# mit-acl/mppi_numba

Measured on AMD Instinct MI355X. Metric: rollouts/sec (MPPI iteration = noise + rollout + update), higher is better.
Workload: dtype f64 intermediates / f32 state (the reference CPU path's roundings)

## Files before the change

### include/mppi_hip.h

```cpp
#ifndef MPPI_HIP_H
#define MPPI_HIP_H

#include <stdint.h>

#ifdef __cplusplus
extern "C" {
#endif

#define MPPI_HIP_ABI_VERSION 1

typedef enum mppi_status {
  MPPI_OK = 0,
  MPPI_ERR_INVALID = -1,
  MPPI_ERR_HIP = -2,
  MPPI_ERR_STATE = -3,
  MPPI_ERR_NO_DEVICE = -4,
  MPPI_ERR_COMM = -5,
  MPPI_ERR_BUSY = -6
} mppi_status;

typedef enum mppi_mode {
  MPPI_MODE_DET = 0,
  MPPI_MODE_SPEED_MAP = 1,
  MPPI_MODE_TDM = 2,
// ... 166 lines not shown
int mppi_planner_time_kernels(mppi_planner* p, mppi_tdm* lin, mppi_tdm* ang, int reps, float* us_rollout,
                              float* us_update);
int mppi_planner_last_elapsed_ms(mppi_planner* p, float* ms);

int mppi_trace_ranges_enabled(void);

int mppi_planner_describe_last_rollout(mppi_planner* p, char* buf, int capacity);

#define MPPI_DEBUG_NO_SPEC_KERNEL 1
#define MPPI_DEBUG_NO_SPECULATION 2
#define MPPI_DEBUG_NO_DEEP_KERNEL 4
#define MPPI_DEBUG_CC_GLOBAL 8
#define MPPI_DEBUG_KEEP_SPECULATING 16
#define MPPI_DEBUG_NO_SCAN_KERNEL 32
#define MPPI_DEBUG_SCAN_READ_NOISE 64
#define MPPI_DEBUG_SCAN_FULL_TILES 128
#define MPPI_DEBUG_NO_FOLDED_APPLY 256
#define MPPI_DEBUG_NO_REDUCE_FOLD 512
#define MPPI_DEBUG_NO_SCAN_DIRECT 1024
#define MPPI_DEBUG_DROP_NOISE_FLAG 2048
int mppi_planner_set_debug_flags(mppi_planner* p, int flags);
int mppi_planner_set_fold_poll_limit(mppi_planner* p, int polls);
int mppi_planner_fold_state(mppi_planner* p, int* folding, long* faults);
int mppi_debug_occupy_cus(int device, int workgroups, int milliseconds);
int mppi_selftest_philox(int device, int* mismatches);
int mppi_debug_read_stamps(unsigned long long* out, int count, int clear);
int mppi_planner_set_graph_replay(mppi_planner* p, int iterations_per_graph);
int mppi_planner_graph_stats(mppi_planner* p, long* captures, long* replays);
int mppi_planner_graph_probe(mppi_planner* p, mppi_tdm* lin, mppi_tdm* ang, int iterations, int replays,
                             float* us_direct, float* us_graph);

typedef struct mppi_world mppi_world;
int mppi_world_create(int device, int rows, int cols, double res, double xlo, double ylo, const double* lin,
                      const double* ang, mppi_world** out);
int mppi_world_destroy(mppi_world* w);
int mppi_world_get(mppi_world* w, const double* xy, int count, double* lin_out, double* ang_out);
int mppi_world_get_grids(mppi_world* w, double* lin, double* ang);
int mppi_world_sample_true_dist(mppi_world* w, const int32_t* terrain_of_cell, int n_terrains, const double* lin_pool,
                                const double* ang_pool, int pool_len, uint64_t seed);
int mppi_planner_closed_loop(mppi_planner* p, mppi_tdm* lin, mppi_tdm* ang, mppi_world* w, int max_steps,
                             double dt, double goal_tolerance, const double* x_init, double* xhist, float* uhist,
                             int* steps_taken);

#define MPPI_COMM_ID_BYTES 128
int mppi_comm_unique_id(char id[MPPI_COMM_ID_BYTES]);
int mppi_planner_comm_init(mppi_planner* p, const char id[MPPI_COMM_ID_BYTES]);
// ... 25 lines not shown
```

### mppi_numba_amd/_lib.py

```python
import ctypes as C
import os

_HERE = os.path.dirname(os.path.abspath(__file__))
LIB_PATH = os.environ.get("MPPI_HIP_LIB") or os.path.join(_HERE, "libmppi_hip.so")

MPPI_OK = 0
MODE_DET, MODE_SPEED_MAP, MODE_TDM, MODE_BAREBONE = 0, 1, 2, 3
RNG_PHILOX, RNG_XOROSHIRO = 0, 1
MATH_EXACT, MATH_FAST = 0, 1
COMM_ID_BYTES = 128
PREP_TDM, PREP_DET, PREP_SPEED = 0, 1, 2
DEBUG_NO_SPEC_KERNEL, DEBUG_NO_SPECULATION, DEBUG_NO_DEEP_KERNEL, DEBUG_CC_GLOBAL = 1, 2, 4, 8
DEBUG_KEEP_SPECULATING = 16
DEBUG_NO_SCAN_KERNEL, DEBUG_SCAN_READ_NOISE, DEBUG_SCAN_FULL_TILES = 32, 64, 128
DEBUG_NO_FOLDED_APPLY = 256
DEBUG_NO_REDUCE_FOLD = 512
DEBUG_NO_SCAN_DIRECT = 1024
DEBUG_DROP_NOISE_FLAG = 2048
ABI_VERSION = 1
P2P_HANDLE_BYTES = 64


class MppiError(RuntimeError):
    def __init__(self, code, message):
# ... 88 lines not shown
    "mppi_planner_iterate_async": [_vp, _vp, _vp, C.c_int],
    "mppi_planner_synchronize": [_vp],
    "mppi_planner_sample_noise": [_vp],
    "mppi_planner_set_noise": [_vp, _f32p],
    "mppi_planner_get_noise": [_vp, _f32p],
    "mppi_planner_rollout": [_vp, _vp, _vp],
    "mppi_planner_set_costs": [_vp, _f32p],
    "mppi_planner_get_costs": [_vp, _f32p],
    "mppi_planner_get_sample_costs": [_vp, _f32p],
    "mppi_planner_update": [_vp],
    "mppi_planner_get_weights": [_vp, _f32p],
    "mppi_planner_get_state_rollout": [_vp, _vp, _vp, _f32p],
    "mppi_planner_get_instance_state_rollout": [_vp, _vp, _vp, C.c_int, _f32p],
    "mppi_planner_set_instances": [_vp, C.c_int, _f32p, _f32p],
    "mppi_planner_rng_states": [_vp, _u64p, C.c_long, C.POINTER(C.c_long)],
    "mppi_planner_set_profiling": [_vp, C.c_int],
    "mppi_planner_stage_times": [_vp, _f32p],
    "mppi_planner_last_elapsed_ms": [_vp, _f32p],
    "mppi_planner_time_kernels": [_vp, _vp, _vp, C.c_int, _f32p, _f32p],
    "mppi_planner_describe_last_rollout": [_vp, C.c_char_p, C.c_int],
    "mppi_planner_set_debug_flags": [_vp, C.c_int],
    "mppi_planner_set_fold_poll_limit": [_vp, C.c_int],
    "mppi_planner_fold_state": [_vp, C.POINTER(C.c_int), C.POINTER(C.c_long)],
    "mppi_debug_occupy_cus": [C.c_int, C.c_int, C.c_int],
    "mppi_selftest_philox": [C.c_int, C.POINTER(C.c_int)],
    "mppi_debug_read_stamps": [C.POINTER(C.c_ulonglong), C.c_int, C.c_int],
    "mppi_planner_graph_probe": [_vp, _vp, _vp, C.c_int, C.c_int, _f32p, _f32p],
    "mppi_planner_set_graph_replay": [_vp, C.c_int],
    "mppi_planner_graph_stats": [_vp, C.POINTER(C.c_long), C.POINTER(C.c_long)],
    "mppi_planner_p2p_export": [_vp, C.c_char_p],
    "mppi_planner_p2p_connect": [_vp, C.c_char_p, C.c_int],
    "mppi_group_p2p_connect": [C.POINTER(_vp), C.c_int],
    "mppi_planner_p2p_stats": [_vp, C.POINTER(C.c_int), C.POINTER(C.c_long), C.c_char_p, C.c_int],
    "mppi_planner_p2p_set_enabled": [_vp, C.c_int],
    "mppi_planner_p2p_ping": [_vp, C.c_ulonglong, C.c_int, C.POINTER(C.c_int)],
    "mppi_world_create": [C.c_int, C.c_int, C.c_int, C.c_double, C.c_double, C.c_double, _f64p, _f64p, C.POINTER(_vp)],
    "mppi_world_destroy": [_vp],
    "mppi_world_get": [_vp, _f64p, C.c_int, _f64p, _f64p],
    "mppi_world_get_grids": [_vp, _f64p, _f64p],
    "mppi_world_sample_true_dist": [_vp, C.POINTER(C.c_int32), C.c_int, _f64p, _f64p, C.c_int, C.c_uint64],
    "mppi_planner_closed_loop": [_vp, _vp, _vp, _vp, C.c_int, C.c_double, C.c_double, _f64p, _f64p, _f32p, C.POINTER(C.c_int)],
    "mppi_tdm_set_sample_shard": [_vp, C.c_int],
    "mppi_planner_set_sample_sharding": [_vp, C.c_int, C.c_int],
    "mppi_planner_sample_costs_local": [_vp, _f32p],
    "mppi_planner_sample_costs_apply": [_vp, _f32p, C.c_int],
    "mppi_comm_unique_id": [C.c_char_p],
# ... 60 lines not shown
```

### mppi_numba_amd/csrc/handles.h

```cpp
#pragma once
#include "host_common.h"
#include "map_plan.h"

struct mppi_tdm {
  mppi_tdm_cfg cfg;
  hipStream_t stream = nullptr;
  int8_t* grid = nullptr;
  int8_t* pmf = nullptr;
  size_t pmf_capacity = 0;
  int8_t* table = nullptr;
  int table_capacity = 0;
  int8_t* obs = nullptr;
  int8_t* unk = nullptr;
  int8_t* risk = nullptr;
  size_t map_capacity = 0;
  int8_t* raw = nullptr;
  size_t raw_capacity = 0;
  float* bin_values = nullptr;
  int bin_values_capacity = 0;
  int* prep_flags = nullptr;
  uint64_t* states = nullptr;
  long n_states = 0;
  int bins = 0, rows = 0, cols = 0;
  bool has_risk = false, maps_set = false, one_hot = false;
// ... 85 lines not shown
  float2* u = nullptr;
  float2* u_prev = nullptr;
  float2* u_alt = nullptr;
  bool apply_pending = false;
  uint64_t folded_applies = 0;
  float* costs = nullptr;
  float* weights_out = nullptr;
  float* w_rel = nullptr;
  float* tile_beta = nullptr;
  int n_tiles = 0;
  bool tile_packets_fresh = false;
  bool theta_bounded = false;
  float* tile_packets[2] = {nullptr, nullptr};
  int tpk_cur = 0;
  int scan_tile = 32;
  bool scan_packets_fresh = false;
  unsigned long long* published = nullptr;
  unsigned int* fold_fault_host = nullptr;
  unsigned int* fold_fault_dev = nullptr;
  int fold_max_polls = 1 << 20;
  long iterations_since_wait = 0;
  bool fold_off = false;
  uint64_t fold_faults = 0;
  bool reduce_pending = false;
  int reduce_index = 0;
  uint64_t reduced_applies = 0;
  uint64_t bumps_owed = 0;
  bool scan_gen_now = false;
  bool noise_virtual = false;
  int noise_virtual_back = 1;
  double* packets = nullptr;
  double* stats = nullptr;
  uint32_t* cells = nullptr;
  size_t cells_capacity = 0;
  double* cc_scratch = nullptr;
  uint16_t* cells16 = nullptr;
  size_t cells16_capacity = 0;
  int pitch16 = 0;
  bool cells16_valid = false;
  bool cells16_with_risk = false;
  int num_cus = 256;
  int lds_per_cu = 160 * 1024;
  float* sample_costs = nullptr;
  bool want_sample_costs = false;
  uint64_t* states = nullptr;
  long n_states = 0;
// ... 123 lines not shown
```

### mppi_numba_amd/csrc/launch_plan.h

```cpp
#pragma once
#include "handles.h"

static int tdm_max_byte(const mppi_tdm* t) { return t->injected ? (int)t->injected_max : t->table_max; }

static int check_tdms(const mppi_planner* p, const mppi_tdm* lin, const mppi_tdm* ang) {
  if (p->cfg.mode == MPPI_MODE_BAREBONE) return MPPI_OK;
  REQUIRE(lin && ang, MPPI_ERR_INVALID, "lin/ang TDM required in this mode");
  REQUIRE(lin->maps_set && ang->maps_set, MPPI_ERR_STATE, "TDM maps not set");
  REQUIRE(lin->cfg.device == p->cfg.device && ang->cfg.device == p->cfg.device, MPPI_ERR_INVALID,
          "planner and TDMs live on different devices");
  REQUIRE(lin->rows == ang->rows && lin->cols == ang->cols, MPPI_ERR_INVALID,
          "lin and ang TDMs differ in padded size (%dx%d vs %dx%d)", lin->rows, lin->cols, ang->rows,
          ang->cols);
  REQUIRE(lin->cfg.num_grids == p->cfg.num_grid_samples && ang->cfg.num_grids == p->cfg.num_grid_samples,
          MPPI_ERR_INVALID, "TDM num_grids (%d, %d) != planner num_grid_samples (%d)", lin->cfg.num_grids,
          ang->cfg.num_grids, p->cfg.num_grid_samples);
  REQUIRE(lin->cfg.max_rows == ang->cfg.max_rows && lin->cfg.max_cols == ang->cfg.max_cols, MPPI_ERR_INVALID,
          "lin and ang TDMs differ in max_map_dim");
  REQUIRE(p->cfg.mode != MPPI_MODE_SPEED_MAP || lin->has_risk, MPPI_ERR_STATE,
          "speed-map mode needs lin TDM's risk traction map");
  return MPPI_OK;
}

static DevParams make_dev_params(const mppi_planner* p) {
// ... 362 lines not shown
  if (p->apply_pending || p->reduce_pending) {
    const mppi_params& a = p->params;
    pend.packets = p->packets;
    pend.u_out = p->u_alt;
    pend.u_prev = p->u_prev;
    pend.stats = p->stats;
    pend.world = p->cfg.world_size;
    pend.stride = p->B * packet_len(T);
    pend.lambda = a.lambda_weight;
    pend.v_lo = a.vrange[0]; pend.v_hi = a.vrange[1];
    pend.w_lo = a.wrange[0]; pend.w_hi = a.wrange[1];
  }
  if (p->reduce_pending) {
    REQUIRE(!p->apply_pending, MPPI_ERR_STATE, "internal: tile packets left to a launch that cannot reduce them");
    REQUIRE(tiles_can_reduce(tiles, T) && plan.tile == p->scan_tile, MPPI_ERR_STATE, "internal: %d workgroups cannot combine the tile packets of %d steps", tiles, T);
    pend.packets = p->packets;
    pend.world = 1;
    pend.reduce_tiles = p->tile_packets[p->tpk_cur];
    pend.reduce_n_tiles = ceil_div(N, p->scan_tile);
    pend.published = p->published;
    pend.flag_set = p->reduce_index & 1;
    pend.fault = p->fold_fault_dev;
    pend.max_polls = p->fold_max_polls;
    if (p->p2p_on) pend.peers = make_peer_exchange(p);
  }
  if (!plan.direct) p->spec_launches += 1;
  REQUIRE(!plan.direct || plan.fallback_offset >= 0, MPPI_ERR_STATE, "internal: direct exact schedule without its map window");
  const ScanFallback fallback = {plan.fallback_offset, plan.fallback_map_bytes, plan.direct ? 1 : 0, plan.rot_ok ? 1 : 0, plan.small_offset};
#define MPPI_LAUNCH_SCAN_EXACT(P2, GEN)                                                                    \
  do {                                                                                                    \
    auto kern = speed ? k_rollout_scan_exact<P2, GEN, false, true>                                        \
                      : (plan.direct ? k_rollout_scan_exact<P2, GEN, true> : k_rollout_scan_exact<P2, GEN, false>); \
    if (plan.lds > 64 * 1024)                                                                             \
      HIP_TRY(hipFuncSetAttribute(reinterpret_cast<const void*>(kern),                                    \
                                  hipFuncAttributeMaxDynamicSharedMemorySize, (int)plan.lds));            \
    MPPI_KLAUNCH(kern, dim3(tiles), dim3(64 * plan.waves), plan.lds, p->stream, d, p->cells16, p->cells,   \
                 p->noise, gen_job, p->u, p->costs, p->w_rel, pk, pend, fallback,                          \
                 (const int8_t*)(speed ? p->packed.risk : nullptr));                                       \
  } while (0)
#define MPPI_LAUNCH_SCAN(RR, P2, GEN)                                                                      \
  do {                                                                                                    \
    auto kern = k_rollout_scan<RR, P2, GEN>;                                                              \
    if (plan.lds > 64 * 1024)                                                                             \
      HIP_TRY(hipFuncSetAttribute(reinterpret_cast<const void*>(kern),                                    \
                                  hipFuncAttributeMaxDynamicSharedMemorySize, (int)plan.lds));            \
    MPPI_KLAUNCH(kern, dim3(tiles + extra), dim3(64 * plan.waves), plan.lds, p->stream, d, p->cells16,    \
// ... 697 lines not shown
```

### mppi_numba_amd/csrc/mppi_api.hip

```cpp
#include "../../include/mppi_hip.h"

#include <dlfcn.h>
#include <hip/hip_runtime.h>
#include <hip/hip_ext.h>
#include <rccl/rccl.h>

#include <algorithm>
#include <atomic>
#include <cmath>
#include <cstdarg>
#include <cstdio>
#include <cstdlib>
#include <cstring>
#include <ctime>
#include <string>
#include <vector>

#include "rng_kernels.h"
#include "rollout_kernels.h"
#include "rollout_crowd_kernel.h"
#include "fleet_kernels.h"
#include "rollout_scan_kernel.h"
#include "rollout_scan_exact_kernel.h"
#include "map_kernels.h"
// ... 437 lines not shown
  if (p->comm && g_rccl.CommDestroy) (void)g_rccl.CommDestroy(p->comm);
  for (int g = 0; g < kMaxFoldedRanks; ++g)
    if (p->peer_mapped[g] && p->peer_inbox[g]) (void)hipIpcCloseMemHandle(p->peer_inbox[g]);
  if (p->inbox) (void)hipFree(p->inbox);
  if (p->p2p_fault_host) (void)hipHostFree(p->p2p_fault_host);
  if (p->fold_fault_host) (void)hipHostFree(p->fold_fault_host);
  dev_free(p->inst_dev);
  if (p->u_host) (void)hipHostFree(p->u_host);
  if (p->u_stage) (void)hipHostFree(p->u_stage);
  if (p->ev_u_staged) (void)hipEventDestroy(p->ev_u_staged);
  dev_free(p->noise_buf[0]);
  dev_free(p->noise_buf[1]);
  dev_free(p->staging);
  dev_free(p->u);
  dev_free(p->u_prev);
  dev_free(p->u_alt);
  dev_free(p->costs);
  dev_free(p->weights_out);
  dev_free(p->w_rel);
  dev_free(p->tile_beta);
  dev_free(p->tile_packets[0]);
  dev_free(p->tile_packets[1]);
  dev_free(p->published);
  dev_free(p->packets);
  dev_free(p->stats);
  dev_free(p->cells);
  dev_free(p->cells16);
  dev_free(p->cc_scratch);
  dev_free(p->sample_costs);
  dev_free(p->states);
  dev_free(p->obs_pos);
  dev_free(p->obs_r);
  dev_free(p->inst_obs_pos);
  dev_free(p->inst_obs_r);
  dev_free(p->trk_pos);
  dev_free(p->trk_pos_rows);
  dev_free(p->trk_r);
  dev_free(p->wall_seg);
  dev_free(p->wall_hw);
  dev_free(p->wtrk_seg_rows);
  dev_free(p->wtrk_hw);
  dev_free(p->wtrk_range);
  dev_free(p->fleet_seg_rows);
  dev_free(p->fleet_hw);
  dev_free(p->fleet_range);
  dev_free(p->fleet_plan);
// ... 68 lines not shown
  HIP_TRY(hipHostMalloc(reinterpret_cast<void**>(&p->u_host), B * T * sizeof(float2), hipHostMallocMapped));
  HIP_TRY(hipHostGetDevicePointer(reinterpret_cast<void**>(&p->u_host_dev), p->u_host, 0));
  memset(p->u_host, 0, B * T * sizeof(float2));
  HIP_TRY(hipHostMalloc(reinterpret_cast<void**>(&p->u_stage), B * T * sizeof(float2), hipHostMallocDefault));
  HIP_TRY(hipEventCreateWithFlags(&p->ev_u_staged, hipEventDisableTiming));
  p->inst_host.assign(B, BatchInst{});
  TRY(dev_alloc(&p->costs, N));
  TRY(dev_alloc(&p->weights_out, N));
  p->n_tiles = ceil_div((long)N, 64);
  TRY(dev_alloc(&p->w_rel, N));
  TRY(dev_alloc(&p->tile_beta, (size_t)p->n_tiles));
  TRY(dev_alloc(&p->packets, (size_t)c.world_size * B * packet_len((int)T)));
  if (c.mode == MPPI_MODE_DET || c.mode == MPPI_MODE_SPEED_MAP) {
    const size_t tiles = (size_t)ceil_div((long)N, 32);
    for (int b = 0; b < 2; ++b) {
      TRY(dev_alloc(&p->tile_packets[b], tiles * (size_t)tile_packet_floats((int)T)));
      HIP_TRY(hipMemsetAsync(p->tile_packets[b], 0, tiles * (size_t)tile_packet_floats((int)T) * sizeof(float), p->stream));
    }
    TRY(dev_alloc(&p->published, published_words((int)T)));
    HIP_TRY(hipMemsetAsync(p->published, 0xff, sizeof(unsigned long long) * published_words((int)T), p->stream));
    HIP_TRY(hipHostMalloc((void**)&p->fold_fault_host, sizeof(unsigned int), hipHostMallocMapped));
    HIP_TRY(hipHostGetDevicePointer((void**)&p->fold_fault_dev, p->fold_fault_host, 0));
    *p->fold_fault_host = 0u;
  }
  TRY(dev_alloc(&p->stats, 2 * B));
  TRY(dev_alloc(&p->state_rollout, (size_t)c.num_vis_state_rollouts * (T + 1) * 3));
  HIP_TRY(hipMemsetAsync(p->u, 0, B * T * sizeof(float2), p->stream));
  HIP_TRY(hipMemsetAsync(p->u_prev, 0, B * T * sizeof(float2), p->stream));
  HIP_TRY(hipMemsetAsync(p->u_alt, 0, B * T * sizeof(float2), p->stream));
  HIP_TRY(hipMemsetAsync(p->costs, 0, N * sizeof(float), p->stream));
  {
    std::vector<double> initial_stats(2 * B);
    for (size_t b = 0; b < B; ++b) { initial_stats[2 * b] = 0.0; initial_stats[2 * b + 1] = 1.0; }
    HIP_TRY(hipMemcpy(p->stats, initial_stats.data(), sizeof(double) * 2 * B, hipMemcpyHostToDevice));
  }
  if (c.rng == MPPI_RNG_XOROSHIRO) {
    long total = (long)c.num_control_rollouts * (long)B * c.num_steps;
    std::vector<uint64_t> host(2 * (size_t)total);
    xoroshiro_init_host(host.data(), total, c.seed);
    p->n_states = (long)N * (long)T;
    TRY(dev_alloc(&p->states, 2 * (size_t)p->n_states));
    HIP_TRY(hipMemcpy(p->states, host.data() + 2 * (size_t)p->n_offset * T,
                      2 * sizeof(uint64_t) * (size_t)p->n_states, hipMemcpyHostToDevice));
  }
  HIP_TRY(hipStreamSynchronize(p->stream));
  return MPPI_OK;
// ... 242 lines not shown
extern "C" int mppi_planner_synchronize(mppi_planner* p) {
  REQUIRE(p, MPPI_ERR_INVALID, "NULL planner");
  HIP_TRY(hipSetDevice(p->cfg.device));
  TRY(wait_for_stream(p));
  TRY(after_drain(p));
  return finish_timing(p);
}

extern "C" int mppi_planner_set_fold_poll_limit(mppi_planner* p, int polls) {
  REQUIRE(p && polls >= 1, MPPI_ERR_INVALID, "bad argument");
  p->fold_max_polls = polls;
  drop_graphs(p);
  p->fold_off = false;
  return MPPI_OK;
}

extern "C" int mppi_planner_fold_state(mppi_planner* p, int* folding, long* faults) {
  REQUIRE(p && folding && faults, MPPI_ERR_INVALID, "NULL argument");
  *folding = p->fold_off ? 0 : 1;
  *faults = (long)p->fold_faults;
  return MPPI_OK;
}

__global__ __launch_bounds__(64) void k_debug_occupy(unsigned long long ticks, int* sink) {
  extern __shared__ int occupy_lds[];
  occupy_lds[threadIdx.x] = (int)threadIdx.x;
  const unsigned long long t0 = wall_clock64();
  while (wall_clock64() - t0 < ticks) __builtin_amdgcn_s_sleep(32);
  if (sink && occupy_lds[threadIdx.x ^ 1] == -1) *sink = 1;
}

extern "C" int mppi_debug_occupy_cus(int device, int workgroups, int milliseconds) {
  REQUIRE(workgroups >= 1 && workgroups <= 4096 && milliseconds >= 1 && milliseconds <= 2000, MPPI_ERR_INVALID, "bad argument");
  HIP_TRY(hipSetDevice(device));
  static hipStream_t sides[64] = {};
  REQUIRE(device >= 0 && device < 64, MPPI_ERR_INVALID, "device %d", device);
  hipStream_t& side = sides[device];
  if (!side) {
    int least = 0, greatest = 0;
    HIP_TRY(hipDeviceGetStreamPriorityRange(&least, &greatest));
    HIP_TRY(hipStreamCreateWithPriority(&side, hipStreamNonBlocking, greatest));
  }
  int rate_khz = 0;
  HIP_TRY(hipDeviceGetAttribute(&rate_khz, hipDeviceAttributeWallClockRate, device));
  if (rate_khz <= 0) rate_khz = 100000;
  const size_t lds = 100 * 1024;
// ... 1107 lines not shown
```

### mppi_numba_amd/csrc/rollout_scan_exact_kernel.h

```cpp
#pragma once
#include "rollout_scan_kernel.h"

namespace mppi {

#ifndef MPPI_SCAN_POLL_SLEEP
#define MPPI_SCAN_POLL_SLEEP 2
#endif

struct ScanFallback {
  int offset;
  int map_bytes;
  int direct;
  int rot_ok;
  int small_offset;
};
static_assert(ScanFallbackLds::kRingBytes == PipeRing<8>::kBytesPerPair, "the region holds one chunk ring of 8 steps");

template <bool POW2RES, typename Background>
__device__ __forceinline__ float scan_exact_reexecute(const DevParams& P, const uint16_t* __restrict__ cells16, char* fb,
                                                      int map_bytes, const float2* e2, const float2* u_src, int T,
                                                      int c, int lane, const float2* us_ready, bool rot_ok,
                                                      Background&& background, bool leave_when_idle = false) {
  constexpr int C = 8, R = ScanExactLds::R;
  using Ring = PipeRing<C>;
// ... 140 lines not shown
#pragma unroll
  for (int i = 0; i < 16; ++i) {
    g = c == i ? kGroupOfWave[i] : g;
    prio = c == i ? kPrioOfWave[i] : prio;
  }
  g = g < W ? g : -1;
  const int k = 2 * g + h;
  [[maybe_unused]] const bool stamp_wg = blockIdx.x == 5 || blockIdx.x == 200;
  [[maybe_unused]] const int stamp_base = (blockIdx.x == 200 ? 1024 : 64) + 16 * c;
  MPPI_STAMP(stamp_wg && c < 16, stamp_base + 0);
  DevParams Q = P;
  const int tile = blockIdx.x;
  const float2* uq = select_instance(Q, u, Q.inst ? (tile * R) / Q.n_inst : 0);
  const int T = Q.n_steps, N = Q.n_local;
  const int Tp = 8 * W;
  const int n = tile * R + r;
  const bool live = n < N;
  const int t0 = k * CHL;
  const int nvalid = min(max(T - t0, 0), CHL);
  const bool folded = pend.packets != nullptr;
  const bool reducing = folded && pend.reduce_tiles != nullptr;
  const int red_t = tile + max(walker, 0) * (int)gridDim.x;
  const bool reduce_here = reducing && (walker == 0 || walker == 1) && red_t < T;
  StepLoads red_loads;
  float2 red_u = make_float2(0.0f, 0.0f);
  if (reduce_here) {
    red_loads = combine_step_issue(pend.reduce_tiles, pend.reduce_n_tiles, tile_packet_floats(T), red_t, lane);
    red_u = uq[red_t];
  }

  const uint32_t ref = scan_lookup<POW2RES, SPEED>(Q, cells16, Q.x0, Q.y0) & 0x3fffu;

  char* base = reinterpret_cast<char*>(scan_lds);
  constexpr bool direct = DIRECT;
  if (direct && c >= 5)
    copy_window_to_lds_direct(Q, cells16, reinterpret_cast<uint16_t*>(base + fallback.offset + (size_t)Tp * 8), 320, (int)blockDim.x - 320);
  float2* e2 = reinterpret_cast<float2*>(base);
  double* ccr = reinterpret_cast<double*>(base + L::e2(W));
  char* grp = base + L::e2(W) + L::ccr(W);
  float2* pos = reinterpret_cast<float2*>(grp + L::grp(W));
  float* th_sh = reinterpret_cast<float*>(pos) + (size_t)Tp * R;
  char* small = DIRECT ? base + fallback.small_offset : reinterpret_cast<char*>(pos) + L::p2(W);
  double2* uos = reinterpret_cast<double2*>(small);
  double* term_sh = reinterpret_cast<double*>(uos + Tp);
  uint32_t* evw = reinterpret_cast<uint32_t*>(term_sh + R);
  float* wsh = reinterpret_cast<float*>(evw + 2 * R);
  uint32_t* flags = reinterpret_cast<uint32_t*>(wsh + R);
  double* scale_sh = reinterpret_cast<double*>(small + (size_t)Tp * 16 + R * 64 + 64);
  float2* u_sh = reinterpret_cast<float2*>(scale_sh + kMaxFoldedRanks + 2);
  int* a_done = reinterpret_cast<int*>(u_sh + Tp);
  int* th_done = a_done + 16;
  int* b_done = th_done + 16;
  int* xy_done = b_done + 16;
  int* ev_done = xy_done + 16;
  int* c_done = ev_done + 16;
  int* cc_done = c_done + 16;
  int* u_ready = cc_done + 16;
  double2* stop_sh = reinterpret_cast<double2*>(u_ready + 16);
  if (c == 4) {
    if (lane < R) {
      evw[2 * lane] = 0u;
      evw[2 * lane + 1] = 0u;
      if (lane == 0) flags[0] = 0u;
    }
    for (int i = lane; i < 8 * 16; i += 64) a_done[i] = 0;
  }
  if (!reducing || c == 1 || (walker < 0 && g < 0)) {
    if (direct && reducing && c >= 5) asm volatile("s_waitcnt vmcnt(0)" ::: "memory");
    lds_barrier();
  }
  MPPI_STAMP(stamp_wg && c < 16, stamp_base + 9);
  auto raise = [&](int* flag, int value) {
    pin_memory_order();
    if (lane == 0) __hip_atomic_store(flag, value, __ATOMIC_RELAXED, __HIP_MEMORY_SCOPE_WORKGROUP);
    pin_memory_order();
  };
  auto peek = [&](const int* flag) {
    return __builtin_amdgcn_readfirstlane(__hip_atomic_load(flag, __ATOMIC_ACQUIRE, __HIP_MEMORY_SCOPE_WORKGROUP));
  };
#ifdef MPPI_POLL_BOUND
  constexpr int kMaxPolls = 1 << 19;
#endif
  auto wait_for = [&](const int* flag) {
    int v;
    [[maybe_unused]] int polls = 0;
    while ((v = peek(flag)) == 0) {
      __builtin_amdgcn_s_sleep(MPPI_SCAN_POLL_SLEEP);
#ifdef MPPI_POLL_BOUND
      if (++polls > kMaxPolls) __builtin_trap();
#endif
    }
    return v;
  };
  const double dt64 = (double)Q.dt;

  if (folded && (walker == 0 || walker == 1)) {
    __builtin_amdgcn_s_setprio(3);
    if (reducing) {
      MPPI_STAMP(stamp_wg, stamp_base + 5);
      if (reduce_here) {
        const int stride = tile_packet_floats(T);
        publish_step(pend, combine_step_finish(red_loads, pend.reduce_tiles, pend.reduce_n_tiles, stride, red_t, pend.lambda, lane),
                     red_u, red_t, T, lane);
        for (int tt = red_t + 2 * (int)gridDim.x; tt < T; tt += 2 * (int)gridDim.x)
          publish_step(pend, combine_step(pend.reduce_tiles, pend.reduce_n_tiles, stride, tt, pend.lambda, lane), uq[tt], tt, T, lane);
      }
      MPPI_STAMP(stamp_wg, stamp_base + 6);
      if (walker == 0) collect_published(pend, T, Tp, lane, u_sh);
      MPPI_STAMP(stamp_wg, stamp_base + 7);
      lds_barrier();
    } else if (walker == 0) {
      pending_apply_prepare(pend, lane, scale_sh);
      pin_memory_order();
      for (int tt = lane; tt < Tp; tt += 64) {
        const float2 v = tt < T ? pending_apply_control(pend, scale_sh, uq, tt) : make_float2(0.0f, 0.0f);
        u_sh[tt] = v;
        if (tile == 0 && tt < T) {
          pend.u_out[tt] = v;
          pend.u_prev[tt] = v;
        }
      }
      if (tile == 0 && lane == 0) {
        pend.stats[0] = scale_sh[kMaxFoldedRanks + 1];
        pend.stats[1] = scale_sh[kMaxFoldedRanks];
      }
    }
    if (walker == 0 && !reducing) raise(&u_ready[0], 1);
  }

  auto glance = [&](const int* flag) {
    return __hip_atomic_load(flag, __ATOMIC_RELAXED, __HIP_MEMORY_SCOPE_WORKGROUP);
  };
  auto settle = [&](int raw) {
// ... 478 lines not shown
```

### mppi_numba_amd/csrc/update_kernels.h

```cpp
#pragma once
#include "device_math.h"
#include "lds_layouts.h"

namespace mppi {

constexpr int kUpdateThreads = 256;

__host__ __device__ inline int packet_len(int n_steps) { return 2 + 2 * n_steps; }

__device__ __forceinline__ float2 updated_control(float2 ut, double nx, double ny, double den, float v_lo,
                                                  float v_hi, float w_lo, float w_hi) {
  ut.x = clip_f32(ut.x + (float)(nx / den), v_lo, v_hi);
  ut.y = clip_f32(ut.y + (float)(ny / den), w_lo, w_hi);
  return ut;
}

__device__ __forceinline__ void apply_update(float2* u, float2* u_prev, float2* u_mirror, int t, double nx,
                                             double ny, double den, float v_lo, float v_hi, float w_lo,
                                             float w_hi) {
  const float2 ut = updated_control(u[t], nx, ny, den, v_lo, v_hi, w_lo, w_hi);
  u[t] = ut;
  u_prev[t] = ut;
  if (u_mirror) u_mirror[t] = ut;
}
// ... 19 lines not shown
  for (int polls = 0; polls < max_polls; ++polls) {
    const bool got = lane < X.world && __hip_atomic_load(const_cast<unsigned long long*>(own) + lane, __ATOMIC_RELAXED,
                                                         __HIP_MEMORY_SCOPE_SYSTEM) == token;
    heard = __popcll(__ballot(got));
    if (heard == X.world) break;
    __builtin_amdgcn_s_sleep(16);
  }
  if (lane == 0) *result = heard;
}

struct PendingApply {
  const double* packets;
  float2* u_out;
  float2* u_prev;
  double* stats;
  int world, stride;
  float lambda, v_lo, v_hi, w_lo, w_hi;
  const float* reduce_tiles;
  int reduce_n_tiles;
  unsigned long long* published;
  int flag_set;
  unsigned int* fault;
  int max_polls;
  PeerExchange peers;
};

__host__ __device__ inline int tile_packet_floats(int n_steps) { return 2 + 2 * n_steps; }

__device__ __forceinline__ void pending_apply_prepare(const PendingApply& A, int lane, double* scale_sh) {
  const double mine = A.packets[(size_t)min(lane, A.world - 1) * A.stride];
  double beta = A.packets[0];
  for (int g = 1; g < A.world; ++g) beta = fmin(beta, A.packets[(size_t)g * A.stride]);
  const double neg_inv_lambda = -1.0 / (double)A.lambda;
  if (lane < A.world) scale_sh[lane] = exp(neg_inv_lambda * (mine - beta));
  if (lane == 0) {
    double den = 0.0;
    for (int g = 0; g < A.world; ++g) den += scale_sh[g] * A.packets[(size_t)g * A.stride + 1];
    scale_sh[kMaxFoldedRanks] = den;
    scale_sh[kMaxFoldedRanks + 1] = beta;
  }
}

__device__ __forceinline__ float2 pending_apply_control(const PendingApply& A, const double* scale_sh,
                                                        const float2* __restrict__ u_old, int t) {
  double nx = 0.0, ny = 0.0;
  for (int g = 0; g < A.world; ++g) {
// ... 169 lines not shown
          all_there = all_there && w[q] != kNotPublished;
        }
      }
      if (__all(all_there)) break;
      if (polls > limit || ((polls & 255) == 255 && A.fault &&
                            __hip_atomic_load(A.fault, __ATOMIC_RELAXED, __HIP_MEMORY_SCOPE_SYSTEM) != 0u)) {
        if (!A.fault) __builtin_trap();
        if (lane == 0) __hip_atomic_store(A.fault, 1u, __ATOMIC_RELAXED, __HIP_MEMORY_SCOPE_SYSTEM);
#pragma unroll
        for (int q = 0; q < 2; ++q) {
          const int t = base + lane + 64 * q;
          if (t < n_steps && w[q] == kNotPublished) w[q] = published_word(A.u_out[t]);
        }
        break;
      }
      __builtin_amdgcn_s_sleep(1);
    }
#pragma unroll
    for (int q = 0; q < 2; ++q) {
      const int t = base + lane + 64 * q;
      if (t < padded_steps)
        u_sh[t] = t < n_steps ? make_float2(__uint_as_float((unsigned int)w[q]), __uint_as_float((unsigned int)(w[q] >> 32)))
                              : make_float2(0.0f, 0.0f);
    }
  }
}

__device__ __forceinline__ void emit_tile_weights(float cost, bool live, float lambda, int n, int tile,
                                                  float* __restrict__ w_rel, float* __restrict__ tile_beta) {
  float beta = wave_min_f32(live ? cost : __builtin_inff());
  if (live) w_rel[n] = (float)exp(-1.0 / (double)lambda * (double)(cost - beta));
  if ((threadIdx.x & 63) == 0) tile_beta[tile] = beta;
}

__global__ __launch_bounds__(64) void k_tile_weights(const float* __restrict__ costs, int n, float lambda,
                                                     float* __restrict__ w_rel, float* __restrict__ tile_beta) {
  int i = blockIdx.x * 64 + threadIdx.x;
  bool live = i < n;
  emit_tile_weights(live ? costs[i] : 0.0f, live, lambda, i, blockIdx.x, w_rel, tile_beta);
}

constexpr int kRowThreads = 1024;

template <bool APPLY, int TC, bool FROM_COSTS = false, int THREADS = kRowThreads>
__global__ __launch_bounds__(THREADS) void k_update_rows(const float* __restrict__ w_rel,
                                                             const float* __restrict__ tile_beta, int n, int n_tiles,
// ... 282 lines not shown
```

### mppi_numba_amd/mppi.py

```python
#!/usr/bin/env python3
import copy
import ctypes as C
import time

import numpy as np

from . import _lib
from .device_array import DeviceArray

DEFAULT_UNKNOWN_COST = float(1e2)
DEFAULT_OBS_COST = float(1e5)
DEFAULT_DIST_WEIGHT = 1.0


def _f32(values):
    return np.asarray(values, dtype=np.float64).astype(np.float32)


class MPPI_Numba(object):


    def __init__(self, cfg, rank=0, world_size=1, sample_shard=None):
        self.cfg = cfg
        for name in ("T", "dt", "num_steps", "num_grid_samples", "num_control_rollouts",
# ... 327 lines not shown
    def iterate_async(self, iterations):
        _lib.call("mppi_planner_iterate_async", self._handle, self.lin_tdm._handle,
                  self.ang_tdm._handle, int(iterations))

    def synchronize(self):
        _lib.call("mppi_planner_synchronize", self._handle)

    def last_rollout_kernel(self):
        buf = C.create_string_buffer(512)
        _lib.call("mppi_planner_describe_last_rollout", self._handle, buf, 512)
        return buf.value.decode()

    def set_debug_flags(self, flags):
        _lib.call("mppi_planner_set_debug_flags", self._handle, int(flags))

    def set_fold_poll_limit(self, polls):
        _lib.call("mppi_planner_set_fold_poll_limit", self._handle, int(polls))

    def fold_state(self):
        folding, faults = C.c_int(0), C.c_long(0)
        _lib.call("mppi_planner_fold_state", self._handle, C.byref(folding), C.byref(faults))
        return bool(folding.value), int(faults.value)

    def set_graph_replay(self, enabled=True, iterations_per_graph=2):
        _lib.call("mppi_planner_set_graph_replay", self._handle, int(iterations_per_graph) if enabled else 0)

    def graph_stats(self):
        captures, replays = C.c_long(0), C.c_long(0)
        _lib.call("mppi_planner_graph_stats", self._handle, C.byref(captures), C.byref(replays))
        return dict(captures=int(captures.value), replays=int(replays.value))

    def set_profiling(self, enabled):
        _lib.call("mppi_planner_set_profiling", self._handle, int(bool(enabled)))

    def stage_times_ms(self):
        ms = (C.c_float * 4)()
        _lib.call("mppi_planner_stage_times", self._handle, ms)
        return dict(noise=ms[0], rollout=ms[1], update=ms[2], collective=ms[3])

    def last_elapsed_ms(self):
        ms = C.c_float(0)
        _lib.call("mppi_planner_last_elapsed_ms", self._handle, C.byref(ms))
        return float(ms.value)

    def comm_init(self, unique_id):
        assert len(unique_id) == _lib.COMM_ID_BYTES
# ... 117 lines not shown
```

Baseline: 565.0 million.

## Fold sparse tile weights locally in walker zero instead of per-step publish

When few tiles carry non-negligible weight, walker 0 gathers only those tiles' packets and computes every step's updated control itself, using a tree-ordered stack summation in double. It then records the results into the published words, replacing the per-step combine and publish across workgroups followed by collection. This targets the cross-workgroup reduction and polling in the folded update path. It adds debug counters written by one thread without atomics, a probe kernel, and an extra poll on published words, with possible rounding-order differences versus the dense path.

```diff
diff --git a/include/mppi_hip.h b/include/mppi_hip.h
--- a/include/mppi_hip.h
+++ b/include/mppi_hip.h
@@ -212,6 +212,9 @@
 int mppi_planner_set_debug_flags(mppi_planner* p, int flags);
 int mppi_planner_set_fold_poll_limit(mppi_planner* p, int polls);
 int mppi_planner_fold_state(mppi_planner* p, int* folding, long* faults);
+int mppi_planner_fold_stats(mppi_planner* p, long* sparse, long* published, int* most_tiles, int* sparse_max);
+int mppi_debug_fold_probe(int device, const float* tile_packets, int n_tiles, int n_steps, const float* u_old, float lambda,
+                          const float* vrange, const float* wrange, float* u_full, float* u_head, int* path);
 int mppi_debug_occupy_cus(int device, int workgroups, int milliseconds);
 int mppi_selftest_philox(int device, int* mismatches);
 int mppi_debug_read_stamps(unsigned long long* out, int count, int clear);
diff --git a/mppi_numba_amd/_lib.py b/mppi_numba_amd/_lib.py
--- a/mppi_numba_amd/_lib.py
+++ b/mppi_numba_amd/_lib.py
@@ -134,6 +134,8 @@
     "mppi_planner_set_debug_flags": [_vp, C.c_int],
     "mppi_planner_set_fold_poll_limit": [_vp, C.c_int],
     "mppi_planner_fold_state": [_vp, C.POINTER(C.c_int), C.POINTER(C.c_long)],
+    "mppi_planner_fold_stats": [_vp, C.POINTER(C.c_long), C.POINTER(C.c_long), C.POINTER(C.c_int), C.POINTER(C.c_int)],
+    "mppi_debug_fold_probe": [C.c_int, _f32p, C.c_int, C.c_int, _f32p, C.c_float, _f32p, _f32p, _f32p, _f32p, C.POINTER(C.c_int)],
     "mppi_debug_occupy_cus": [C.c_int, C.c_int, C.c_int],
     "mppi_selftest_philox": [C.c_int, C.POINTER(C.c_int)],
     "mppi_debug_read_stamps": [C.POINTER(C.c_ulonglong), C.c_int, C.c_int],
diff --git a/mppi_numba_amd/csrc/handles.h b/mppi_numba_amd/csrc/handles.h
--- a/mppi_numba_amd/csrc/handles.h
+++ b/mppi_numba_amd/csrc/handles.h
@@ -131,6 +131,7 @@
   long iterations_since_wait = 0;
   bool fold_off = false;
   uint64_t fold_faults = 0;
+  unsigned int* fold_words = nullptr;
   bool reduce_pending = false;
   int reduce_index = 0;
   uint64_t reduced_applies = 0;
diff --git a/mppi_numba_amd/csrc/launch_plan.h b/mppi_numba_amd/csrc/launch_plan.h
--- a/mppi_numba_amd/csrc/launch_plan.h
+++ b/mppi_numba_amd/csrc/launch_plan.h
@@ -408,6 +408,7 @@
     pend.flag_set = p->reduce_index & 1;
     pend.fault = p->fold_fault_dev;
     pend.max_polls = p->fold_max_polls;
+    pend.fold_words = p->fold_words;
     if (p->p2p_on) pend.peers = make_peer_exchange(p);
   }
   if (!plan.direct) p->spec_launches += 1;
diff --git a/mppi_numba_amd/csrc/mppi_api.hip b/mppi_numba_amd/csrc/mppi_api.hip
--- a/mppi_numba_amd/csrc/mppi_api.hip
+++ b/mppi_numba_amd/csrc/mppi_api.hip
@@ -483,6 +483,7 @@
   dev_free(p->tile_packets[0]);
   dev_free(p->tile_packets[1]);
   dev_free(p->published);
+  dev_free(p->fold_words);
   dev_free(p->packets);
   dev_free(p->stats);
   dev_free(p->cells);
@@ -597,6 +598,8 @@
     HIP_TRY(hipHostMalloc((void**)&p->fold_fault_host, sizeof(unsigned int), hipHostMallocMapped));
     HIP_TRY(hipHostGetDevicePointer((void**)&p->fold_fault_dev, p->fold_fault_host, 0));
     *p->fold_fault_host = 0u;
+    TRY(dev_alloc(&p->fold_words, (size_t)4));
+    HIP_TRY(hipMemsetAsync(p->fold_words, 0, 4 * sizeof(unsigned int), p->stream));
   }
   TRY(dev_alloc(&p->stats, 2 * B));
   TRY(dev_alloc(&p->state_rollout, (size_t)c.num_vis_state_rollouts * (T + 1) * 3));
@@ -885,6 +888,92 @@
   return MPPI_OK;
 }
 
+extern "C" int mppi_planner_fold_stats(mppi_planner* p, long* sparse, long* published, int* most_tiles, int* sparse_max) {
+  REQUIRE(p && sparse && published && most_tiles && sparse_max, MPPI_ERR_INVALID, "NULL argument");
+  HIP_TRY(hipSetDevice(p->cfg.device));
+  TRY(drain_stream(p));
+  unsigned int words[4] = {0u, 0u, 0u, 0u};
+  if (p->fold_words) HIP_TRY(hipMemcpy(words, p->fold_words, sizeof(words), hipMemcpyDeviceToHost));
+  *sparse = (long)words[0];
+  *published = (long)words[1];
+  *most_tiles = (int)words[2];
+  *sparse_max = kFoldSparseMax;
+  return MPPI_OK;
+}
+
+__global__ __launch_bounds__(64) void k_debug_fold_probe(const float* __restrict__ tile_packets, int n_tiles, int n_steps,
+                                                         const float2* __restrict__ u_old, PendingApply A,
+                                                         float2* __restrict__ u_full, float2* __restrict__ u_head,
+                                                         int* __restrict__ path) {
+  extern __shared__ double2 probe_lds[];
+  const int lane = threadIdx.x, stride = tile_packet_floats(n_steps), padded = (n_steps + 7) & ~7;
+  float2* u_sh = reinterpret_cast<float2*>(probe_lds);
+  char* scratch = reinterpret_cast<char*>(u_sh + padded);
+  for (int t = 0; t < n_steps; ++t) {
+    const StepSums S = combine_step(tile_packets, n_tiles, stride, t, A.lambda, lane);
+    if (lane == 0) u_full[t] = updated_control(u_old[t], S.nx, S.ny, S.den, A.v_lo, A.v_hi, A.w_lo, A.w_hi);
+  }
+  FoldHead H = fold_head_issue(tile_packets, n_tiles, stride, lane);
+  const FoldScales F = fold_scales(H, n_tiles, A.lambda, lane);
+  const bool went_sparse = F.count <= kFoldSparseMax && n_tiles <= 256;
+  if (went_sparse) {
+    (void)fold_sparse_combine(A, H, F, tile_packets, stride, n_steps, padded, u_old, u_sh, scratch, lane);
+    __syncthreads();
+    for (int t = lane; t < n_steps; t += 64) u_head[t] = u_sh[t];
+  } else {
+    for (int t = 0; t < n_steps; ++t) {
+      const StepSums S = combine_step(tile_packets, n_tiles, stride, t, A.lambda, lane);
+      if (lane == 0) u_head[t] = updated_control(u_old[t], S.nx, S.ny, S.den, A.v_lo, A.v_hi, A.w_lo, A.w_hi);
+    }
+  }
+  if (lane == 0) {
+    path[0] = went_sparse ? 1 : 0;
+    path[1] = F.count;
+  }
+}
+
+extern "C" int mppi_debug_fold_probe(int device, const float* tile_packets, int n_tiles, int n_steps, const float* u_old,
+                                     float lambda, const float* vrange, const float* wrange, float* u_full, float* u_head,
+                                     int* path) {
+  REQUIRE(tile_packets && u_old && vrange && wrange && u_full && u_head && path, MPPI_ERR_INVALID, "NULL argument");
+  REQUIRE(n_tiles >= 1 && n_tiles <= 4096 && n_steps >= 1 && n_steps <= 128 && lambda > 0.0f, MPPI_ERR_INVALID, "bad argument");
+  HIP_TRY(hipSetDevice(device));
+  const size_t floats = (size_t)n_tiles * tile_packet_floats(n_steps);
+  float* d_packets = nullptr;
+  float2 *d_old = nullptr, *d_out = nullptr;
+  int* d_path = nullptr;
+  int rc = MPPI_OK;
+  auto body = [&]() -> int {
+    TRY(dev_alloc(&d_packets, floats));
+    TRY(dev_alloc(&d_old, (size_t)n_steps));
+    TRY(dev_alloc(&d_out, (size_t)2 * n_steps));
+    TRY(dev_alloc(&d_path, (size_t)2));
+    HIP_TRY(hipMemcpy(d_packets, tile_packets, floats * sizeof(float), hipMemcpyHostToDevice));
+    HIP_TRY(hipMemcpy(d_old, u_old, (size_t)n_steps * sizeof(float2), hipMemcpyHostToDevice));
+    PendingApply A;
+    memset(&A, 0, sizeof(A));
+    A.lambda = lambda;
+    A.v_lo = vrange[0]; A.v_hi = vrange[1];
+    A.w_lo = wrange[0]; A.w_hi = wrange[1];
+    const int padded = (n_steps + 7) & ~7;
+    const size_t lds = (size_t)padded * sizeof(float2) + fold_sparse_lds_bytes(padded < 64 ? padded : 64);
+    hipLaunchKernelGGL(k_debug_fold_probe, dim3(1), dim3(64), lds, 0, d_packets, n_tiles, n_steps, d_old, A, d_out,
+                       d_out + n_steps, d_path);
+    HIP_TRY(hipGetLastError());
+    HIP_TRY(hipDeviceSynchronize());
+    HIP_TRY(hipMemcpy(u_full, d_out, (size_t)n_steps * sizeof(float2), hipMemcpyDeviceToHost));
+    HIP_TRY(hipMemcpy(u_head, d_out + n_steps, (size_t)n_steps * sizeof(float2), hipMemcpyDeviceToHost));
+    HIP_TRY(hipMemcpy(path, d_path, 2 * sizeof(int), hipMemcpyDeviceToHost));
+    return MPPI_OK;
+  };
+  rc = body();
+  dev_free(d_packets);
+  dev_free(d_old);
+  dev_free(d_out);
+  dev_free(d_path);
+  return rc;
+}
+
 __global__ __launch_bounds__(64) void k_debug_occupy(unsigned long long ticks, int* sink) {
   extern __shared__ int occupy_lds[];
   occupy_lds[threadIdx.x] = (int)threadIdx.x;
diff --git a/mppi_numba_amd/csrc/rollout_scan_exact_kernel.h b/mppi_numba_amd/csrc/rollout_scan_exact_kernel.h
--- a/mppi_numba_amd/csrc/rollout_scan_exact_kernel.h
+++ b/mppi_numba_amd/csrc/rollout_scan_exact_kernel.h
@@ -186,9 +186,15 @@
   const bool reducing = folded && pend.reduce_tiles != nullptr;
   const int red_t = tile + max(walker, 0) * (int)gridDim.x;
   const bool reduce_here = reducing && (walker == 0 || walker == 1) && red_t < T;
+  constexpr bool kFoldLocal = !DIRECT;
+  const bool fold_local = kFoldLocal && reducing && walker == 0;
   StepLoads red_loads;
+  FoldHead fold_head;
   float2 red_u = make_float2(0.0f, 0.0f);
-  if (reduce_here) {
+  if (fold_local) {
+    fold_head = fold_head_issue(pend.reduce_tiles, pend.reduce_n_tiles, tile_packet_floats(T), lane);
+    if (red_t < T) red_u = uq[red_t];
+  } else if (reduce_here) {
     red_loads = combine_step_issue(pend.reduce_tiles, pend.reduce_n_tiles, tile_packet_floats(T), red_t, lane);
     red_u = uq[red_t];
   }
@@ -232,6 +238,15 @@
   if (!reducing || c == 1 || (walker < 0 && g < 0)) {
     if (direct && reducing && c >= 5) asm volatile("s_waitcnt vmcnt(0)" ::: "memory");
     lds_barrier();
+    if (kFoldLocal && reducing && c == 1) {
+      const bool went_sparse = scale_sh[0] != 0.0;
+      if (tile == 0 && lane == 0 && pend.fold_words) {
+        const unsigned int carrying = (unsigned int)scale_sh[1];
+        pend.fold_words[went_sparse ? 0 : 1] += 1u;
+        if (carrying > pend.fold_words[2]) pend.fold_words[2] = carrying;
+      }
+      if (went_sparse) watch_published(pend, T, lane);
+    }
   }
   MPPI_STAMP(stamp_wg && c < 16, stamp_base + 9);
   auto raise = [&](int* flag, int value) {
@@ -262,6 +277,29 @@
     __builtin_amdgcn_s_setprio(3);
     if (reducing) {
       MPPI_STAMP(stamp_wg, stamp_base + 5);
+      bool went_sparse = false;
+      float fold_beta = 0.0f;
+      double fold_den = 0.0;
+      if (fold_local) {
+        const int stride = tile_packet_floats(T);
+        const FoldScales F = fold_scales(fold_head, pend.reduce_n_tiles, pend.lambda, lane);
+        went_sparse = F.count <= kFoldSparseMax && pend.reduce_n_tiles <= 256 && pend.peers.world == 0;
+        if (lane == 0) {
+          scale_sh[0] = went_sparse ? 1.0 : 0.0;
+          scale_sh[1] = (double)F.count;
+        }
+        if (went_sparse) {
+          fold_beta = F.beta;
+          fold_den = fold_sparse_combine(pend, fold_head, F, pend.reduce_tiles, stride, T, Tp, uq, u_sh, grp, lane);
+        } else if (reduce_here) {
+          red_loads = combine_step_issue(pend.reduce_tiles, pend.reduce_n_tiles, stride, red_t, lane);
+        }
+      }
+      if (went_sparse) {
+        MPPI_STAMP(stamp_wg, stamp_base + 7);
+        lds_barrier();
+        for (int tt = red_t; tt < T; tt += 2 * (int)gridDim.x) fold_sparse_record(pend, u_sh, fold_beta, fold_den, tt, T, lane);
+      } else {
       if (reduce_here) {
         const int stride = tile_packet_floats(T);
         publish_step(pend, combine_step_finish(red_loads, pend.reduce_tiles, pend.reduce_n_tiles, stride, red_t, pend.lambda, lane),
@@ -273,6 +311,7 @@
       if (walker == 0) collect_published(pend, T, Tp, lane, u_sh);
       MPPI_STAMP(stamp_wg, stamp_base + 7);
       lds_barrier();
+      }
     } else if (walker == 0) {
       pending_apply_prepare(pend, lane, scale_sh);
       pin_memory_order();
diff --git a/mppi_numba_amd/csrc/update_kernels.h b/mppi_numba_amd/csrc/update_kernels.h
--- a/mppi_numba_amd/csrc/update_kernels.h
+++ b/mppi_numba_amd/csrc/update_kernels.h
@@ -65,6 +65,7 @@
   int flag_set;
   unsigned int* fault;
   int max_polls;
+  unsigned int* fold_words;
   PeerExchange peers;
 };
 
@@ -280,6 +281,198 @@
       if (t < padded_steps)
         u_sh[t] = t < n_steps ? make_float2(__uint_as_float((unsigned int)w[q]), __uint_as_float((unsigned int)(w[q] >> 32)))
                               : make_float2(0.0f, 0.0f);
+    }
+  }
+}
+
+constexpr int kFoldSparseMax = 16;
+constexpr int kFoldSparseBatch = 8;
+constexpr int kFoldStackDepth = 6;
+__host__ __device__ inline size_t fold_sparse_lds_bytes(int lanes) {
+  return (size_t)lanes * (kFoldStackDepth * 5 * 8 + kFoldSparseBatch * 2 * 8);
+}
+
+struct FoldHead {
+  float2 bd[4];
+};
+__device__ __forceinline__ FoldHead fold_head_issue(const float* __restrict__ tile_packets, int n_tiles, int stride, int lane) {
+  FoldHead H;
+#pragma unroll
+  for (int q = 0; q < 4; ++q)
+    H.bd[q] = *reinterpret_cast<const float2*>(tile_packets + (size_t)min(lane + 64 * q, n_tiles - 1) * stride);
+  return H;
+}
+struct FoldScales {
+  float beta;
+  float s[4];
+  unsigned long long present[4];
+  int count;
+};
+__device__ __forceinline__ FoldScales fold_scales(FoldHead& H, int n_tiles, float lambda, int lane) {
+  FoldScales F;
+#pragma unroll
+  for (int q = 0; q < 4; ++q)
+    if (lane + 64 * q >= n_tiles) H.bd[q] = make_float2(__builtin_inff(), 0.0f);
+  F.beta = wave_min_f32(fminf(fminf(H.bd[0].x, H.bd[1].x), fminf(H.bd[2].x, H.bd[3].x)));
+  const float beta = F.beta;
+  const float scale = -1.4426950408889634f / lambda;
+  F.count = 0;
+#pragma unroll
+  for (int q = 0; q < 4; ++q) {
+    const float tb = H.bd[q].x == __builtin_inff() ? beta : H.bd[q].x;
+    F.s[q] = __builtin_amdgcn_exp2f((tb - beta) * scale);
+    F.present[q] = __ballot(lane + 64 * q < n_tiles && !(F.s[q] == 0.0f));
+    F.count += __popcll(F.present[q]);
+  }
+  return F;
+}
+struct FoldTileIter {
+  unsigned long long lanes;
+  unsigned int slots;
+  int lane;
+  __device__ __forceinline__ explicit FoldTileIter(const FoldScales& F)
+      : lanes(F.present[0] | F.present[1] | F.present[2] | F.present[3]), slots(0u), lane(0) {}
+  __device__ __forceinline__ int next_slot(const FoldScales& F) {
+    if (slots == 0u) {
+      lane = __builtin_ctzll(lanes);
+      lanes &= lanes - 1ull;
+      slots = (unsigned int)((F.present[0] >> lane) & 1ull) | (unsigned int)((F.present[1] >> lane) & 1ull) << 1 |
+              (unsigned int)((F.present[2] >> lane) & 1ull) << 2 | (unsigned int)((F.present[3] >> lane) & 1ull) << 3;
+    }
+    const int q = __builtin_ctz(slots);
+    slots &= slots - 1u;
+    return q;
+  }
+};
+__device__ __forceinline__ int fold_merge_level(int a, int b) {
+  const int x = a ^ b;
+  return x >= 16 ? 4 : 31 - __builtin_clz((unsigned int)x);
+}
+__device__ __forceinline__ double fold_sparse_combine(const PendingApply& A, const FoldHead& H, const FoldScales& F,
+                                                      const float* __restrict__ tile_packets, int stride, int n_steps,
+                                                      int padded_steps, const float2* __restrict__ u_old, float2* u_sh,
+                                                      char* scratch, int lane) {
+  const int lanes = min(64, padded_steps);
+  const bool act = lane < lanes, two = padded_steps > 64;
+  double* stack = reinterpret_cast<double*>(scratch);
+  float2* stage = reinterpret_cast<float2*>(stack + kFoldStackDepth * 5 * lanes);
+  const int t0 = min(lane, n_steps - 1), t1 = min(lane + 64, n_steps - 1);
+  const float2 uo0 = u_old[t0], uo1 = u_old[t1];
+  double top[5] = {0.0, 0.0, 0.0, 0.0, 0.0};
+  int top_lane = -1, sp = 0;
+  unsigned long long reps = 0ull;
+  auto pop_into_top = [&]() {
+    --sp;
+    reps >>= 8;
+    if (act) {
+#pragma unroll
+      for (int v = 0; v < 5; ++v) top[v] = stack[(sp * 5 + v) * lanes + lane] + top[v];
+    }
+  };
+  FoldTileIter issue(F), walk(F);
+  for (int done = 0; done < F.count; done += kFoldSparseBatch) {
+    const int cnt = min(F.count - done, kFoldSparseBatch);
+    float2 m[kFoldSparseBatch][2];
+#pragma unroll
+    for (int i = 0; i < kFoldSparseBatch; ++i) {
+      if (i < cnt) {
+        const int q = issue.next_slot(F);
+        const float* at = tile_packets + (size_t)(issue.lane + 64 * q) * stride + 2;
+        m[i][0] = *reinterpret_cast<const float2*>(at + 2 * t0);
+        m[i][1] = two ? *reinterpret_cast<const float2*>(at + 2 * t1) : make_float2(0.0f, 0.0f);
+      }
+    }
+#pragma unroll
+    for (int i = 0; i < kFoldSparseBatch; ++i) {
+      if (i < cnt && act) {
+        stage[(2 * i) * lanes + lane] = m[i][0];
+        stage[(2 * i + 1) * lanes + lane] = m[i][1];
+      }
+    }
+    for (int i = 0; i < cnt; ++i) {
+      const int q = walk.next_slot(F);
+      const int l = walk.lane;
+      const float sq = q == 0 ? F.s[0] : (q == 1 ? F.s[1] : (q == 2 ? F.s[2] : F.s[3]));
+      const float dq = q == 0 ? H.bd[0].y : (q == 1 ? H.bd[1].y : (q == 2 ? H.bd[2].y : H.bd[3].y));
+      const double s = (double)__int_as_float(__builtin_amdgcn_readlane(__float_as_int(sq), l));
+      const double td = (double)__int_as_float(__builtin_amdgcn_readlane(__float_as_int(dq), l));
+      float2 a = make_float2(0.0f, 0.0f), b = a;
+      if (act) {
+        a = stage[(2 * i) * lanes + lane];
+        b = stage[(2 * i + 1) * lanes + lane];
+      }
+      if (l != top_lane) {
+        if (top_lane >= 0) {
+          const int level = fold_merge_level(top_lane, l);
+          while (sp > 0 && fold_merge_level((int)(reps & 63ull), top_lane) <= level) pop_into_top();
+          if (act) {
+#pragma unroll
+            for (int v = 0; v < 5; ++v) stack[(sp * 5 + v) * lanes + lane] = top[v];
+          }
+          reps = (reps << 8) | (unsigned long long)top_lane;
+          ++sp;
+#pragma unroll
+          for (int v = 0; v < 5; ++v) top[v] = 0.0;
+        }
+        top_lane = l;
+      }
+      top[0] = fma(s, (double)a.x, top[0]);
+      top[1] = fma(s, (double)a.y, top[1]);
+      top[2] = fma(s, (double)b.x, top[2]);
+      top[3] = fma(s, (double)b.y, top[3]);
+      top[4] = fma(s, td, top[4]);
+    }
+  }
+  while (sp > 0) pop_into_top();
+  const double den = __longlong_as_double(
+      ((long long)__builtin_amdgcn_readfirstlane((int)(__double_as_longlong(top[4]) >> 32)) << 32) |
+      (unsigned int)__builtin_amdgcn_readfirstlane((int)__double_as_longlong(top[4])));
+  if (lane < padded_steps)
+    u_sh[lane] = lane < n_steps ? updated_control(uo0, top[0], top[1], den, A.v_lo, A.v_hi, A.w_lo, A.w_hi) : make_float2(0.0f, 0.0f);
+  if (lane + 64 < padded_steps)
+    u_sh[lane + 64] = lane + 64 < n_steps ? updated_control(uo1, top[2], top[3], den, A.v_lo, A.v_hi, A.w_lo, A.w_hi) : make_float2(0.0f, 0.0f);
+  return den;
+}
+
+__device__ __forceinline__ void fold_sparse_record(const PendingApply& A, const float2* u_sh, float beta, double den,
+                                                   int tt, int n_steps, int lane) {
+  if (lane == 0) {
+    const float2 ut = u_sh[tt];
+    unsigned long long* mine = A.published + ((size_t)A.flag_set * n_steps + tt) * kPublishedStride;
+    unsigned long long* other = A.published + ((size_t)(A.flag_set ^ 1) * n_steps + tt) * kPublishedStride;
+    __hip_atomic_store(mine, published_word(ut), __ATOMIC_RELAXED, __HIP_MEMORY_SCOPE_AGENT);
+    other[0] = kNotPublished;
+    A.u_out[tt] = ut;
+    A.u_prev[tt] = ut;
+    if (tt == 0) {
+      A.stats[0] = (double)beta;
+      A.stats[1] = den;
+    }
+  }
+}
+
+__device__ __forceinline__ void watch_published(const PendingApply& A, int n_steps, int lane) {
+  unsigned long long* words = A.published + (size_t)A.flag_set * n_steps * kPublishedStride;
+  const int limit = max(A.max_polls, 1);
+  for (int base = 0; base < n_steps; base += 128) {
+    bool seen[2] = {false, false};
+    for (int polls = 0;; ++polls) {
+      bool all_there = true;
+#pragma unroll
+      for (int q = 0; q < 2; ++q) {
+        const int t = base + lane + 64 * q;
+        if (t < n_steps && !seen[q]) {
+          seen[q] = __hip_atomic_load(words + (size_t)t * kPublishedStride, __ATOMIC_RELAXED, __HIP_MEMORY_SCOPE_AGENT) != kNotPublished;
+          all_there = all_there && seen[q];
+        }
+      }
+      if (__all(all_there)) break;
+      if (polls > limit || ((polls & 255) == 255 && A.fault &&
+                            __hip_atomic_load(A.fault, __ATOMIC_RELAXED, __HIP_MEMORY_SCOPE_SYSTEM) != 0u)) {
+        if (A.fault && lane == 0) __hip_atomic_store(A.fault, 1u, __ATOMIC_RELAXED, __HIP_MEMORY_SCOPE_SYSTEM);
+        return;
+      }
+      __builtin_amdgcn_s_sleep(8);
     }
   }
 }
diff --git a/mppi_numba_amd/mppi.py b/mppi_numba_amd/mppi.py
--- a/mppi_numba_amd/mppi.py
+++ b/mppi_numba_amd/mppi.py
@@ -373,6 +373,12 @@
         _lib.call("mppi_planner_fold_state", self._handle, C.byref(folding), C.byref(faults))
         return bool(folding.value), int(faults.value)
 
+    def fold_stats(self):
+        sparse, published, most, limit = C.c_long(0), C.c_long(0), C.c_int(0), C.c_int(0)
+        _lib.call("mppi_planner_fold_stats", self._handle, C.byref(sparse), C.byref(published), C.byref(most), C.byref(limit))
+        return {"sparse": int(sparse.value), "published": int(published.value), "most_tiles": int(most.value),
+                "sparse_max": int(limit.value)}
+
     def set_graph_replay(self, enabled=True, iterations_per_graph=2):
         _lib.call("mppi_planner_set_graph_replay", self._handle, int(iterations_per_graph) if enabled else 0)
 
```

Result: slower. 493.2 million (-12.7%).
